# bcgsc/NanoSim

Hardware: NVIDIA H100
Metric: simulated_bases_per_sec (higher is better)
Workload: dtype u8

## Files before the change

### nanosim_b200/csrc/plan_kernel.cuh

```cuda
#pragma once
#include "device_common.cuh"

struct PlanArgs {
    DevModel m;
    DevRef ref;
    DevCfg cfg;
    uint32_t kind;
    uint64_t first_id;
    uint32_t n_reads;
    const uint32_t* n_seg;
    const uint32_t* piece_first;
    NsReadMeta* reads;
    NsPieceMeta* pieces;
    uint32_t* ops;
    const uint32_t* order;
    uint32_t* counter;
    uint32_t* n_flagged;
    uint32_t batch_reversed;
    const uint32_t* abort;
};

#define NS_MAX_SAME_LEN_RETRIES 64

enum Phase : int { PH_FETCH = 0, PH_LEN, PH_ATT, PH_PIECE, PH_EVENT, PH_UEVENT, PH_PIECE_END, PH_CHECK, PH_DONE };
// ... 94 lines not shown
}

__device__ __forceinline__ void draw_position_meta(const DevRef& ref, Rng& rng, int species, uint32_t length, uint32_t& chrom,
                                                   uint32_t& pos) {
    uint32_t sp = species >= 0 ? (uint32_t)species : (uint32_t)__umul64hi(rng.next64(), (uint64_t)ref.n_species);
    const uint32_t c0 = __ldg(&ref.species_chrom_off[sp]), c1 = __ldg(&ref.species_chrom_off[sp + 1]);
    uint32_t c = c0 + (uint32_t)__umul64hi(rng.next64(), (uint64_t)(c1 - c0));
    uint64_t clen = __ldg(&ref.chrom_off[c + 1]) - __ldg(&ref.chrom_off[c]);
    if ((uint64_t)length > clen) {
        uint32_t n_same = 0, n_all = 0;
        for (uint32_t q = 0; q < ref.n_chrom; ++q) {
            const uint64_t l = __ldg(&ref.chrom_off[q + 1]) - __ldg(&ref.chrom_off[q]);
            if ((uint64_t)length < l) {
                ++n_all;
                if (q >= c0 && q < c1) ++n_same;
            }
        }
        const bool same = n_same > 0;
        const uint32_t n_pick = same ? n_same : n_all - n_same;
        if (n_pick > 0) {
            uint32_t r = (uint32_t)__umul64hi(rng.next64(), (uint64_t)n_pick);
            for (uint32_t q = 0; q < ref.n_chrom; ++q) {
                const uint64_t l = __ldg(&ref.chrom_off[q + 1]) - __ldg(&ref.chrom_off[q]);
                const bool in_sp = q >= c0 && q < c1;
                if ((uint64_t)length < l && in_sp == same) {
                    if (r == 0) {
                        c = q;
                        break;
                    }
                    --r;
                }
            }
            clen = __ldg(&ref.chrom_off[c + 1]) - __ldg(&ref.chrom_off[c]);
        }
    }
    chrom = c;
    if (__ldg(&ref.chrom_circular[c])) {
        pos = (uint32_t)__umul64hi(rng.next64(), clen + 1);
    } else {
        pos = clen >= length ? (uint32_t)__umul64hi(rng.next64(), clen - length + 1) : 0u;
    }
}

__device__ __forceinline__ void draw_position_trx(const DevRef& ref, uint32_t n_records, Rng& rng, uint32_t length, uint32_t& chrom,
                                                  uint32_t& pos) {
    if (ref.trx_len_sorted && ref.n_trx_sorted == n_records) {
        uint32_t lo = 0, hi = n_records;
        while (lo < hi) {
            const uint32_t mid = (lo + hi) >> 1;
            if (__ldg(&ref.trx_len_sorted[mid]) > length) hi = mid; else lo = mid + 1;
        }
        if (lo < n_records) {
            const uint32_t j = lo + (uint32_t)__umul64hi(rng.next64(), (uint64_t)(n_records - lo));
            chrom = __ldg(&ref.trx_len_idx[j]);
            pos = (uint32_t)__umul64hi(rng.next64(), (uint64_t)(__ldg(&ref.trx_len_sorted[j]) - length + 1u));
            return;
        }
        chrom = 0;
        pos = 0;
        return;
    }
    for (int it = 0; it < 1000000; ++it) {
        const uint32_t c = (uint32_t)__umul64hi(rng.next64(), (uint64_t)n_records);
        const uint64_t clen = __ldg(&ref.chrom_off[c + 1]) - __ldg(&ref.chrom_off[c]);
        if ((uint64_t)length < clen) {
            chrom = c;
            pos = (uint32_t)__umul64hi(rng.next64(), clen - length + 1);
            return;
        }
    }
    chrom = 0;
    pos = 0;
}

__device__ __forceinline__ uint32_t lower_bound_f(const float* x, uint32_t n, float v) {
    uint32_t lo = 0, hi = n;
    while (lo < hi) {
        uint32_t mid = (lo + hi) >> 1;
        if (__ldg(&x[mid]) < v) lo = mid + 1; else hi = mid;
    }
    return lo;
}
__device__ __forceinline__ uint32_t nearest_aligned_length(const DevModel& m, uint32_t n_sample, uint32_t L, Rng& rng) {
    const uint32_t M = m.n_kde2d;
    const double u = u01_double(rng.next64());
    const double q = -expm1(log1p(-u) / (double)(n_sample > 0 ? n_sample : 1));
    const double need = q * (double)M;
    const float fl = (float)L;
    const float xmin = __ldg(&m.kde2d_x[0]), xmax = __ldg(&m.kde2d_x[M - 1]);
    uint32_t dlo = 0, dhi = (uint32_t)fmaxf(fabsf(fl - xmin), fabsf(xmax - fl)) + 1;
    while (dlo < dhi) {
        const uint32_t d = (dlo + dhi) >> 1;
        const uint32_t a = lower_bound_f(m.kde2d_x, M, fl - (float)d);
        const uint32_t b = lower_bound_f(m.kde2d_x, M, fl + (float)d + 0.5f);
        if ((double)(b - a) >= need && b > a) dhi = d; else dlo = d + 1;
    }
    const uint32_t d = dlo;
    const uint32_t a0 = lower_bound_f(m.kde2d_x, M, fl - (float)d), a1 = lower_bound_f(m.kde2d_x, M, fl - (float)d + 0.5f);
    uint32_t b0 = 0, b1 = 0;
    if (d > 0) {
        b0 = lower_bound_f(m.kde2d_x, M, fl + (float)d);
        b1 = lower_bound_f(m.kde2d_x, M, fl + (float)d + 0.5f);
    }
    const uint32_t cnt = (a1 - a0) + (b1 - b0);
    uint32_t r = (uint32_t)__umul64hi(rng.next64(), (uint64_t)(cnt > 0 ? cnt : 1));
    const uint32_t row = cnt == 0 ? (a0 < M ? a0 : M - 1) : (r < a1 - a0 ? a0 + r : b0 + (r - (a1 - a0)));
    const uint32_t r1 = rng.next(), r2 = rng.next();
    const float z = sqrtf(-2.0f * logf(u01_open_low(r1))) * cospif(2.0f * ((float)(r2 >> 8) * (1.0f / 16777216.0f)));
    const double y = (double)__ldg(&m.kde2d_y[row]) + (double)m.kde2d_bw * (double)z;
    return y > 0.0 ? (uint32_t)y : 0u;
}

__device__ __forceinline__ void draw_lengths(const DevModel& m, const DevCfg& cfg, uint32_t kind, uint64_t rid, uint32_t gen,
                                             uint32_t n_seg, NsPieceMeta* pieces) {
    Rng lr;
    lr.init(cfg.seed, rid, stream_word(ST_LEN, kind, gen));
    for (uint32_t s = 0; s < n_seg; ++s) {
        uint32_t len = 0;
        for (int it = 0; it < 100000; ++it) {
            double x;
            if (cfg.median_len > 0.0) {
                if (cfg.perfect) {
                    x = lognormal_draw(log(cfg.median_len), cfg.sd_len, lr);
                } else {
                    double t = lognormal_draw(log(cfg.median_len + cfg.sd_len * cfg.sd_len / 2.0), cfg.sd_len, lr);
                    double rem = -1.0;
                    for (int jt = 0; jt < 100000 && rem < 0.0; ++jt) rem = pow(10.0, kde_draw(m.ht, lr)) - 1.0;
                    x = t - rem;
                }
            } else {
                x = kde_draw(m.aligned, lr);
            }
            bool ok = cfg.perfect ? (x >= (double)cfg.min_len && x <= (double)cfg.max_len)
                                  : (x > 0.0 && x <= (double)cfg.max_len);
            if (cfg.metagenome) {
                if (ok) {
                    len = (uint32_t)rint(x);
                    break;
                }
                continue;
            }
            if (ok && (uint32_t)x > 0) {
                len = (uint32_t)x;
                break;
            }
        }
        pieces[2 * s].ref_req = len;
        if (s + 1 < n_seg) {
            double g = pow(10.0, kde_draw(m.gap, lr)) - 1.0;
            int64_t gi = (int64_t)g;
            pieces[2 * s + 1].ref_req = gi > 0 ? (uint32_t)gi : 0u;
        }
    }
}

__global__ void lengths_kernel(DevModel m, DevCfg cfg, uint32_t kind, uint64_t first_id, uint32_t n, const uint32_t* n_seg,
                               const uint32_t* piece_first, NsPieceMeta* pieces, float ev_per_base, float ev_cv, uint32_t exact_only,
                               uint64_t* caps, uint32_t* keys, uint32_t* vals) {
    uint32_t i = blockIdx.x * blockDim.x + threadIdx.x;
    if (i >= n) return;
    const uint32_t ns = n_seg ? n_seg[i] : 1u;
    const uint32_t pf = piece_first ? piece_first[i] : i;
    uint64_t total = 0;
    if (kind == NS_KIND_ALIGNED && cfg.transcriptome) {
        caps[pf] = 0;
    } else if (kind == NS_KIND_ALIGNED) {
        draw_lengths(m, cfg, kind, first_id + i, 0, ns, pieces + pf);
        for (uint32_t q = 0; q < 2 * ns - 1; ++q) {
            const uint32_t len = pieces[pf + q].ref_req;
            total += len;
            uint64_t cap;
            if (q & 1u) cap = 2ull * len + 64;
            else if (cfg.perfect) cap = 4;
            else {
                float e = (float)len * ev_per_base;
                cap = (uint64_t)(2.0f * (e + 6.0f * ev_cv * sqrtf(e) + 8.0f)) + 4;
            }
            caps[pf + q] = exact_only ? 0 : cap;
        }
    } else if (exact_only) {
        caps[pf] = 0;
    } else {
        Rng r0;
        r0.init(cfg.seed, first_id + i, stream_word(ST_ATT, NS_KIND_UNALIGNED, 0));
        const double x = cfg.median_len > 0.0 ? lognormal_draw(log(cfg.median_len), cfg.sd_len, r0) : kde_draw(m.unaligned, r0);
        const uint64_t len = x >= 1.0 ? (x < 268435455.0 ? (uint64_t)x : 268435455ull) : 0ull;
        caps[pf] = len + (len >> 1) + 64;
        total = len;
    }
    keys[i] = total > 0xffffffffull ? 0xffffffffu : (uint32_t)total;
    vals[i] = i;
}

#ifndef PLAN_MIN_BLOCKS
#define PLAN_MIN_BLOCKS 4
#endif
template <bool REPLAY>
__global__ void __launch_bounds__(128, PLAN_MIN_BLOCKS) plan_kernel(const __grid_constant__ PlanArgs a) {
    const DevModel& m = a.m;
    const DevCfg& cfg = a.cfg;
    const bool unal_kind = (a.kind == NS_KIND_UNALIGNED);
    if (a.abort && *a.abort) return;
    __shared__ uint8_t bin_lut[BIN_LUT_SIZE];
    __shared__ uint32_t s_tab_off[NS_MAX_TABLES], s_tab_n[NS_MAX_TABLES], s_trans[NS_N_ERR_STATES * 3];
    for (uint32_t i = threadIdx.x; i < BIN_LUT_SIZE; i += blockDim.x) bin_lut[i] = (uint8_t)match_bin_scan(m, i);
    for (uint32_t i = threadIdx.x; i < NS_MAX_TABLES; i += blockDim.x) {
        s_tab_off[i] = m.tab_off[i];
        s_tab_n[i] = m.tab_n[i];
    }
    for (uint32_t i = threadIdx.x; i < NS_N_ERR_STATES * 3; i += blockDim.x) s_trans[i] = m.trans[i / 3][i % 3];
    __syncthreads();

    int phase = PH_FETCH;
    uint32_t slot = 0;
    uint64_t rid = 0;
    uint32_t n_seg = 1, n_pieces = 1, piece_first = 0;
    uint32_t attempt = 0, gen = 0, gen_fails = 0;
    Rng rng;
    uint32_t remainder = 0, head = 0, tail = 0, reversed = 0;
    uint64_t total = 0, actual = 0;
    uint32_t p = 0;
    uint32_t pos = 0, middle_ref = 0, prev_match = 0, err_state = 0, last_err = 3;
    int64_t l_new = 0;
    uint32_t pending_ins = 0;
    uint4 ev_r = make_uint4(0, 0, 0, 0);
    uint32_t gap_sw = 0, gap_draw = 0;
    bool last_op_was_ins_same_pos = false;
    uint32_t last_ins_len = 0;
    OpSink<true> sink;
    sink.begin(nullptr, 0);
    bool overflow = false;

    for (;;) {
        switch (phase) {
        case PH_FETCH: {
            slot = atomicAdd(a.counter, 1u);
            if (slot >= a.n_reads) {
                phase = PH_DONE;
                break;
            }
            if (a.order) slot = a.order[slot];
            if (REPLAY && !(a.reads[slot].flags & 1u)) break;
            rid = a.first_id + slot;
            n_seg = a.n_seg ? a.n_seg[slot] : 1u;
            piece_first = a.piece_first ? a.piece_first[slot] : slot;
            n_pieces = unal_kind ? 1u : 2u * n_seg - 1u;
            overflow = false;
            if (REPLAY) {
                attempt = a.reads[slot].attempts;
            } else {
                attempt = 0;
                gen = 0;
                gen_fails = 0;
            }
            phase = PH_ATT;
            break;
        }
        case PH_LEN: {
            draw_lengths(m, cfg, a.kind, rid, gen, n_seg, a.pieces + piece_first);
            phase = PH_ATT;
            break;
        }
        case PH_ATT: {
            rng.init(cfg.seed, rid, stream_word(ST_ATT, a.kind, attempt));
            overflow = false;
            p = 0;
            total = 0;
            actual = 0;
            if (unal_kind) {
                double x = cfg.median_len > 0.0 ? lognormal_draw(log(cfg.median_len), cfg.sd_len, rng)
                                                : kde_draw(m.unaligned, rng);
                int64_t r = (int64_t)x;
                if (!REPLAY) a.pieces[piece_first].ref_req = r > 0 ? (uint32_t)r : 0u;
                head = tail = 0;
                remainder = 0;
                if (r <= 0 && !REPLAY) {
                    ++attempt;
                    break;
                }
            } else if (cfg.transcriptome) {
                uint32_t trx = 0, tlen = 0, alen = 0;
                for (int it = 0; it < 1000000; ++it) {
                    const uint32_t r = rng.next();
                    const uint64_t pp = (uint64_t)r * a.ref.n_expressed;
                    const uint32_t j = (uint32_t)(pp >> 32);
                    const uint2 e = __ldg(&a.ref.expr_alias[j]);
                    const uint32_t k = ((uint32_t)pp < e.x || e.x == 0xffffffffu) ? j : e.y;
                    trx = __ldg(&a.ref.expr_chrom[k]);
                    tlen = (uint32_t)(__ldg(&a.ref.chrom_off[trx + 1]) - __ldg(&a.ref.chrom_off[trx]));
                    alen = nearest_aligned_length(m, cfg.kde2d_n, tlen, rng);
                    if (alen < tlen) break;
                }
                NsPieceMeta& pm0 = a.pieces[piece_first];
                pm0.ref_req = alen;
                pm0.chrom = trx;
                reversed = u01_double(rng.next64()) > (double)m.strandness;
                head = tail = 0;
                remainder = 0;
                if (!cfg.perfect) {
                    Rng hr;
                    hr.init(cfg.seed, rid, stream_word(ST_LEN, a.kind, 0));
                    const double rem = pow(10.0, kde_draw(m.ht, hr)) - 1.0;
                    double ratio = kde_draw(m.ratio, hr);
                    ratio = ratio > 1.0 ? 1.0 : (ratio < 0.0 ? 0.0 : ratio);
                    remainder = rem > 0.0 ? (uint32_t)rem : 0u;
                    if (remainder > 0) {
                        head = (uint32_t)rint((double)remainder * ratio);
                        tail = remainder - head;
                    }
                }
            } else if (cfg.perfect) {
                head = tail = 0;
                remainder = 0;
                reversed = u01_double(rng.next64()) > (double)m.strandness;
                if (cfg.metagenome) reversed = a.batch_reversed;
            } else {
                double rem = -1.0;
                for (int it = 0; it < 100000 && rem < 0.0; ++it) rem = pow(10.0, kde_draw(m.ht, rng)) - 1.0;
                double ratio = -1.0;
                for (int it = 0; it < 100000 && (ratio < 0.0 || ratio > 1.0); ++it) ratio = kde_draw(m.ratio, rng);
                remainder = cfg.metagenome ? (uint32_t)rint(rem) : (uint32_t)rem;
                reversed = u01_double(rng.next64()) > (double)m.strandness;
                if (cfg.metagenome) reversed = a.batch_reversed;
                if (remainder == 0) {
                    head = tail = 0;
                } else {
                    head = (uint32_t)rint((double)remainder * ratio);
                    tail = remainder - head;
                }
                total = remainder;
            }
            phase = PH_PIECE;
            break;
        }
        case PH_PIECE: {
            NsPieceMeta& pm = a.pieces[piece_first + p];
            uint32_t m_ref = pm.ref_req;
            sink.begin(a.ops + pm.op_off, REPLAY ? 0xffffffffu : (uint32_t)(a.pieces[piece_first + p + 1].op_off - pm.op_off));
            pos = 0;
            middle_ref = m_ref;
            l_new = (int64_t)m_ref;
// ... 297 lines not shown
```

### nanosim_b200/csrc/uread_kernel.cuh

```cuda
#pragma once
#include "device_common.cuh"
#include "emit_kernel.cuh"
#include "plan_kernel.cuh"

struct UreadArgs {
    DevModel m;
    DevRef ref;
    DevCfg cfg;
    uint64_t first_id;
    uint32_t n_reads;
    NsReadMeta* reads;
    NsPieceMeta* pieces;
    uint32_t* ops;
    const uint32_t* order;
    uint32_t* counter;
    uint32_t* n_flagged;
    unsigned long long* pool_cursor;
    const uint64_t* pool;
    const uint32_t* abort;
    uint32_t cta_min_len;
};

#define UREAD_WARPS 8

__device__ __forceinline__ void scan_advance_and_insertions(bool nonins, uint32_t s, int lane, uint32_t& adv_incl, uint32_t& ins_incl) {
    if (__all_sync(0xffffffffu, s < 2048u)) {
        const uint32_t both = warp_incl_scan(nonins ? s : (s << 16), lane);
        adv_incl = both & 0xffffu;
        ins_incl = both >> 16;
    } else {
        adv_incl = warp_incl_scan(nonins ? s : 0u, lane);
        ins_incl = warp_incl_scan(nonins ? 0u : s, lane);
    }
}

struct UChain {
    uint32_t n_ops, middle_ref, n_draws;
    int64_t l_new;
};
__device__ __forceinline__ UChain unaligned_chain_warp(const DevModel& m, uint2 key, uint32_t id_lo, uint32_t id_hi, uint32_t sw,
                                                       uint32_t m_ref, uint32_t* ops, uint32_t cap, int lane) {
    const uint32_t lane_lt = (1u << lane) - 1u;
    uint32_t base = 0, pos_base = 0, carry_a = 0, middle_ref = m_ref, n_draws = 0, n_ops = 0;
    int64_t l_new = (int64_t)m_ref;
    bool done = false;
    auto draw = [&](uint32_t d, uint32_t& kd, uint32_t& sd) {
        const uint4 r = philox4x32_10(make_uint4(id_lo, id_hi, sw, d + 1u), key);
        kd = r.x < 1717986918u ? 0u : (r.x < 3006477107u ? 1u : (r.x < 3650722201u ? 2u : 3u));
        sd = 1;
        if (kd != 0) sd = alias_draw(m, kd == 1 ? 1u : (kd == 2 ? 2u : 3u), r.y);
    };
    uint32_t kind_next, s_next;
    draw(lane, kind_next, s_next);
    while (!done) {
        const uint32_t kind = kind_next, s = s_next;
        draw(base + 32u + lane, kind_next, s_next);
        const bool nonins = kind != 2;
        uint32_t Pl, I;
        scan_advance_and_insertions(nonins, s, lane, Pl, I);
        const uint32_t P = pos_base + Pl;
        const uint32_t stop_mask = __ballot_sync(0xffffffffu, nonins && P >= m_ref);
        const int jstop = stop_mask ? __ffs(stop_mask) - 1 : 32;
        const bool valid = lane <= jstop;
        const uint32_t nonins_mask = __ballot_sync(0xffffffffu, nonins);
        const uint32_t below = nonins_mask & lane_lt;
        const int pn = below ? 31 - __clz(below) : -1;
        const uint32_t I_pn = __shfl_sync(0xffffffffu, I, pn < 0 ? 0 : pn);
        const uint32_t a_ins = nonins ? (pn >= 0 ? I - I_pn : I + carry_a) : 0u;
        int32_t delta = 0;
        if (valid) delta = kind == 2 ? (int32_t)s : (kind == 3 ? -(int32_t)s : 0);
        delta = __reduce_add_sync(0xffffffffu, delta);
        l_new += delta;

        uint32_t o0 = 0, o1 = 0, o2 = 0, o3 = 0;
        const bool emits = valid && nonins;
        const uint32_t plain_mask = __ballot_sync(0xffffffffu, emits && kind == 0 && a_ins == 0);
        if (emits) {
            if (kind == 0) {
                if (a_ins == 0) {
                    if (!(lane > 0 && ((plain_mask >> (lane - 1)) & 1u))) {
                        const uint32_t run = __ffs(~(plain_mask >> lane)) - 1;
                        o0 = (NS_OP_COPY << 28) | (run == 0xffffffffu ? 32u - lane : run);
                    }
                } else {
                    o0 = (NS_OP_COPY << 28) | 1u;
                    o1 = (NS_OP_INS << 28) | a_ins;
                }
            } else {
                const uint32_t covered = a_ins < s - 1 ? a_ins : s - 1;
                const uint32_t rest = s - 1 - covered;
                const uint32_t T = kind == 1 ? NS_OP_MIS : NS_OP_DEL;
                const uint32_t n_ins = kind == 1 ? a_ins : a_ins - covered;
                if (n_ins == 0) {
                    o0 = (T << 28) | (1u + rest);
                } else {
                    o0 = (T << 28) | 1u;
                    o1 = (NS_OP_INS << 28) | n_ins;
                    if (rest) o2 = (T << 28) | rest;
                }
                if (covered) o3 = (NS_OP_COPY << 28) | covered;
            }
        }
        const uint32_t p1 = o0 ? 1u : 0u, p2 = p1 + (o1 ? 1u : 0u), p3 = p2 + (o2 ? 1u : 0u);
        const uint32_t cnt = p3 + (o3 ? 1u : 0u);
        const uint32_t incl = warp_incl_scan(cnt, lane);
        const uint32_t at = n_ops + incl - cnt;
        if (o0 && at < cap) ops[at] = o0;
        if (o1 && at + p1 < cap) ops[at + p1] = o1;
        if (o2 && at + p2 < cap) ops[at + p2] = o2;
        if (o3 && at + p3 < cap) ops[at + p3] = o3;
        n_ops += __shfl_sync(0xffffffffu, incl, 31);

        if (jstop < 32) {
            const uint32_t Pstop = __shfl_sync(0xffffffffu, P, jstop);
            if (Pstop > middle_ref) {
                l_new += Pstop - middle_ref;
                middle_ref = Pstop;
            }
            n_draws = base + (uint32_t)jstop + 1u;
            done = true;
        } else {
            pos_base = __shfl_sync(0xffffffffu, P, 31);
            const uint32_t I31 = __shfl_sync(0xffffffffu, I, 31);
            if (nonins_mask) {
                const int last = 31 - __clz(nonins_mask);
                carry_a = I31 - __shfl_sync(0xffffffffu, I, last);
            } else {
                carry_a += I31;
            }
            base += 32;
        }
    }
    UChain c;
    c.n_ops = n_ops;
    c.middle_ref = middle_ref;
    c.n_draws = n_draws;
    c.l_new = l_new;
    return c;
}


struct UCtaShared {
    uint32_t A[2][UREAD_WARPS], I[2][UREAD_WARPS], non[2][UREAD_WARPS], trail[2][UREAD_WARPS];
    uint32_t stop[2][UREAD_WARPS], cnt[2][UREAD_WARPS], pstop[2][UREAD_WARPS];
    int32_t delta[2][UREAD_WARPS];
    uint32_t bc32;
    unsigned long long bc64;
};
__device__ __forceinline__ UChain unaligned_chain_cta(const DevModel& m, uint2 key, uint32_t id_lo, uint32_t id_hi, uint32_t sw,
                                                      uint32_t m_ref, uint32_t* ops, uint32_t cap, UCtaShared& sh) {
    const int lane = threadIdx.x & 31, w = threadIdx.x >> 5;
    const uint32_t lane_lt = (1u << lane) - 1u;
    uint32_t base = 0, pos_base = 0, carry_round = 0, middle_ref = m_ref, n_draws = 0, n_ops = 0;
    int64_t l_new = (int64_t)m_ref;
    auto draw = [&](uint32_t d, uint32_t& kd, uint32_t& sd) {
        const uint4 r = philox4x32_10(make_uint4(id_lo, id_hi, sw, d + 1u), key);
        kd = r.x < 1717986918u ? 0u : (r.x < 3006477107u ? 1u : (r.x < 3650722201u ? 2u : 3u));
        sd = 1;
        if (kd != 0) sd = alias_draw(m, kd == 1 ? 1u : (kd == 2 ? 2u : 3u), r.y);
    };
    uint32_t kind_next, s_next;
    draw(32u * (uint32_t)w + lane, kind_next, s_next);
    for (uint32_t par = 0;; par ^= 1u) {
        const uint32_t kind = kind_next, s = s_next;
        draw(base + 32u * UREAD_WARPS + 32u * (uint32_t)w + lane, kind_next, s_next);
        const bool nonins = kind != 2;
        uint32_t Pl, I;
        scan_advance_and_insertions(nonins, s, lane, Pl, I);
        const uint32_t nonins_mask = __ballot_sync(0xffffffffu, nonins);
        const uint32_t P31 = __shfl_sync(0xffffffffu, Pl, 31), I31 = __shfl_sync(0xffffffffu, I, 31);
        const uint32_t I_last = __shfl_sync(0xffffffffu, I, nonins_mask ? 31 - __clz(nonins_mask) : 0);
        if (lane == 0) {
            sh.A[par][w] = P31;
            sh.I[par][w] = I31;
            sh.non[par][w] = nonins_mask != 0u;
            sh.trail[par][w] = nonins_mask ? I31 - I_last : I31;
        }
        __syncthreads();
        uint32_t pos_off = 0, carry_in = carry_round, A_tot = 0, carry_out = carry_round;
#pragma unroll
        for (int v = 0; v < UREAD_WARPS; ++v) {
            const uint32_t Av = sh.A[par][v];
            const uint32_t c = sh.non[par][v] ? sh.trail[par][v] : carry_out + sh.I[par][v];
            if (v < w) {
                pos_off += Av;
                carry_in = c;
            }
            carry_out = c;
            A_tot += Av;
        }
        const uint32_t P = pos_base + pos_off + Pl;
        const uint32_t stop_mask = __ballot_sync(0xffffffffu, nonins && P >= m_ref);
        const int jstop = stop_mask ? __ffs(stop_mask) - 1 : 32;
        const bool valid = lane <= jstop;
        const uint32_t below = nonins_mask & lane_lt;
        const int pn = below ? 31 - __clz(below) : -1;
        const uint32_t I_pn = __shfl_sync(0xffffffffu, I, pn < 0 ? 0 : pn);
        const uint32_t a_ins = nonins ? (pn >= 0 ? I - I_pn : I + carry_in) : 0u;
        int32_t delta = 0;
        if (valid) delta = kind == 2 ? (int32_t)s : (kind == 3 ? -(int32_t)s : 0);
        delta = __reduce_add_sync(0xffffffffu, delta);

        uint32_t o0 = 0, o1 = 0, o2 = 0, o3 = 0;
        const bool emits = valid && nonins;
        const uint32_t plain_mask = __ballot_sync(0xffffffffu, emits && kind == 0 && a_ins == 0);
        if (emits) {
            if (kind == 0) {
                if (a_ins == 0) {
                    if (!(lane > 0 && ((plain_mask >> (lane - 1)) & 1u))) {
                        const uint32_t run = __ffs(~(plain_mask >> lane)) - 1;
                        o0 = (NS_OP_COPY << 28) | (run == 0xffffffffu ? 32u - lane : run);
                    }
                } else {
                    o0 = (NS_OP_COPY << 28) | 1u;
                    o1 = (NS_OP_INS << 28) | a_ins;
                }
            } else {
                const uint32_t covered = a_ins < s - 1 ? a_ins : s - 1;
                const uint32_t rest = s - 1 - covered;
                const uint32_t T = kind == 1 ? NS_OP_MIS : NS_OP_DEL;
                const uint32_t n_ins = kind == 1 ? a_ins : a_ins - covered;
                if (n_ins == 0) {
                    o0 = (T << 28) | (1u + rest);
                } else {
                    o0 = (T << 28) | 1u;
                    o1 = (NS_OP_INS << 28) | n_ins;
                    if (rest) o2 = (T << 28) | rest;
                }
                if (covered) o3 = (NS_OP_COPY << 28) | covered;
            }
        }
        const uint32_t p1 = o0 ? 1u : 0u, p2 = p1 + (o1 ? 1u : 0u), p3 = p2 + (o2 ? 1u : 0u);
        const uint32_t cnt = p3 + (o3 ? 1u : 0u);
        const uint32_t incl = warp_incl_scan(cnt, lane);
        const uint32_t cnt_w = __shfl_sync(0xffffffffu, incl, 31);
        const uint32_t Pstop_w = __shfl_sync(0xffffffffu, P, jstop & 31);
        if (lane == 0) {
            sh.stop[par][w] = (uint32_t)jstop;
            sh.cnt[par][w] = cnt_w;
            sh.delta[par][w] = delta;
            sh.pstop[par][w] = Pstop_w;
        }
        __syncthreads();
        int ws = UREAD_WARPS;
#pragma unroll
        for (int v = UREAD_WARPS - 1; v >= 0; --v)
            if (sh.stop[par][v] < 32u) ws = v;
        uint32_t off = 0, tot = 0;
        int32_t dsum = 0;
#pragma unroll
        for (int v = 0; v < UREAD_WARPS; ++v) {
            if (v <= ws) {
                const uint32_t c = sh.cnt[par][v];
                if (v < w) off += c;
                tot += c;
                dsum += sh.delta[par][v];
            }
        }
        if (w <= ws) {
            const uint32_t at = n_ops + off + incl - cnt;
            if (o0 && at < cap) ops[at] = o0;
            if (o1 && at + p1 < cap) ops[at + p1] = o1;
            if (o2 && at + p2 < cap) ops[at + p2] = o2;
            if (o3 && at + p3 < cap) ops[at + p3] = o3;
        }
        n_ops += tot;
        l_new += dsum;
        if (ws < UREAD_WARPS) {
            const uint32_t Pstop = sh.pstop[par][ws];
            if (Pstop > middle_ref) {
                l_new += Pstop - middle_ref;
                middle_ref = Pstop;
            }
            n_draws = base + 32u * (uint32_t)ws + sh.stop[par][ws] + 1u;
            break;
        }
        pos_base += A_tot;
        carry_round = carry_out;
        base += 32u * UREAD_WARPS;
    }
    UChain c;
    c.n_ops = n_ops;
    c.middle_ref = middle_ref;
    c.n_draws = n_draws;
    c.l_new = l_new;
    return c;
}

#define UREAD_CTA_MIN_LEN 32768u

template <bool REPLAY, bool CTA>
__device__ __forceinline__ uint32_t uread_one(const UreadArgs& a, uint2 key, uint32_t slot, uint64_t pool_base, uint64_t pool_size,
                                              UCtaShared& sh) {
    const DevModel& m = a.m;
    const DevCfg& cfg = a.cfg;
    const int lane = threadIdx.x & 31;
    const bool leader = CTA ? threadIdx.x == 0 : lane == 0;
    const uint64_t rid = a.first_id + slot;
    const uint32_t id_lo = (uint32_t)rid, id_hi = (uint32_t)(rid >> 32);
    uint32_t attempt = REPLAY ? a.reads[slot].attempts : 0u;
    uint64_t op_off = a.pieces[slot].op_off;
    uint32_t* ops = a.ops + op_off;
    uint32_t cap = REPLAY ? 0xffffffffu : (uint32_t)(a.pieces[slot + 1].op_off - op_off);
    uint32_t first_len = 0;
    for (;;) {
        const uint32_t sw = stream_word(ST_ATT, NS_KIND_UNALIGNED, attempt);
        Rng r0;
        r0.init(cfg.seed, rid, sw);
        const double x = cfg.median_len > 0.0 ? lognormal_draw(log(cfg.median_len), cfg.sd_len, r0)
                                              : kde_draw(m.unaligned, r0);
        const int64_t mr = (int64_t)x;
        if (attempt == 0) first_len = mr > 0 ? (uint32_t)mr : 0u;
        if (mr <= 0) {
            ++attempt;
            continue;
        }
        const uint32_t m_ref = (uint32_t)mr;
        if (!REPLAY && attempt > 0) {
            const uint32_t need = m_ref + (m_ref >> 1) + 64u;
            unsigned long long off = 0;
            if (leader) off = atomicAdd(a.pool_cursor, (unsigned long long)need);
            if (CTA) {
                if (leader) sh.bc64 = off;
                __syncthreads();
                off = sh.bc64;
                __syncthreads();
            } else {
                off = __shfl_sync(0xffffffffu, off, 0);
            }
            if (off + need <= pool_size) {
                op_off = pool_base + off;
                cap = need;
            } else {
                cap = 0;
            }
            ops = a.ops + op_off;
        }
        const UChain ch = CTA ? unaligned_chain_cta(m, key, id_lo, id_hi, sw, m_ref, ops, cap, sh)
                              : unaligned_chain_warp(m, key, id_lo, id_hi, sw, m_ref, ops, cap, lane);
        const uint32_t middle_ref = ch.middle_ref, n_draws = ch.n_draws, n_ops = ch.n_ops;
        const int64_t l_new = ch.l_new;
        if (REPLAY) break;
        const bool ok = middle_ref >= cfg.min_len && middle_ref <= cfg.max_len && l_new >= (int64_t)cfg.min_len &&
                        l_new <= (int64_t)cfg.max_len;
        if (!ok) {
            ++attempt;
            continue;
        }
        const uint4 rs = philox4x32_10(make_uint4(id_lo, id_hi, sw, n_draws + 1u), key);
        const uint32_t reversed = u01_double(((uint64_t)rs.x << 32) | rs.y) > (double)m.strandness;
        Rng pr;
        pr.init(cfg.seed, rid, stream_word(ST_POS, NS_KIND_UNALIGNED, attempt));
        uint32_t chrom = 0, ppos = 0;
        if (cfg.metagenome) draw_position_meta(a.ref, pr, -1, middle_ref, chrom, ppos);
        else if (cfg.transcriptome) draw_position_trx(a.ref, cfg.trx_records ? cfg.trx_records : a.ref.n_chrom, pr, middle_ref, chrom, ppos);
        else draw_position(a.ref, cfg, pr, middle_ref, chrom, ppos);
        if (leader) {
            const bool overflow = n_ops > cap;
            NsPieceMeta p;
            p.op_off = op_off;
            p.n_ops = n_ops;
            p.kind = NS_PIECE_UNALIGNED;
            p.chrom = chrom;
            p.pos = ppos;
            p.ref_len = middle_ref;
            p.out_len = (uint32_t)l_new;
            p.out_rel = 0;
            p.l_new = (uint32_t)l_new;
            p.ref_req = m_ref;
            p.read_slot = slot;
            p.ev_off = op_off;
            p.ev_n_ops = n_ops;
            p.polya_len = 0;
            a.pieces[slot] = p;
            NsReadMeta q;
            q.seq_off = 0;
            q.seq_len = (uint32_t)l_new;
            q.head = 0;
            q.tail = 0;
            q.piece_first = slot;
            q.n_pieces = 1;
            q.reversed = (uint8_t)reversed;
            q.flags = overflow ? 1 : 0;
            q.attempts = attempt;
            a.reads[slot] = q;
            if (overflow) atomicAdd(a.n_flagged, 1u);
        }
        break;
    }
    return first_len;
}

#ifndef UREAD_MIN_BLOCKS
#define UREAD_MIN_BLOCKS 3
#endif
template <bool REPLAY>
__global__ void __launch_bounds__(UREAD_WARPS * 32, UREAD_MIN_BLOCKS) uread_kernel(const __grid_constant__ UreadArgs a) {
    const int lane = threadIdx.x & 31;
    const uint2 key = make_uint2((uint32_t)a.cfg.seed, (uint32_t)(a.cfg.seed >> 32));
    if (a.abort && *a.abort) return;
    const uint64_t pool_base = a.pool[0], pool_size = a.pool[1];
    __shared__ UCtaShared sh;

    if (!REPLAY && a.order && a.cta_min_len) {
        for (;;) {
            if (threadIdx.x == 0) sh.bc32 = atomicAdd(a.counter, 1u);
            __syncthreads();
            const uint32_t idx = sh.bc32;
            __syncthreads();
            if (idx >= a.n_reads) return;
            const uint32_t first_len = uread_one<REPLAY, true>(a, key, a.order[idx], pool_base, pool_size, sh);
            if (first_len <= a.cta_min_len) break;
        }
    }
    for (;;) {
        uint32_t idx = 0;
        if (lane == 0) idx = atomicAdd(a.counter, 1u);
        idx = __shfl_sync(0xffffffffu, idx, 0);
        if (idx >= a.n_reads) break;
        const uint32_t slot = a.order ? a.order[idx] : idx;
        if (REPLAY && !(a.reads[slot].flags & 1u)) continue;
        uread_one<REPLAY, false>(a, key, slot, pool_base, pool_size, sh);
    }
}

struct GapArgs {
    DevModel m;
    DevCfg cfg;
    uint32_t kind;
    uint64_t first_id;
    uint32_t n_reads;
    const uint32_t* n_seg;
    const uint32_t* piece_first;
    NsPieceMeta* pieces;
    uint32_t* ops;
    uint32_t* counter;
    const uint32_t* abort;
};
__device__ __forceinline__ uint32_t gap_stream_word(uint32_t kind, uint32_t attempt, uint32_t piece_in_read) {
    return stream_word(ST_GAP, kind, (attempt << 5) | (piece_in_read & 31u));
}
__global__ void __launch_bounds__(UREAD_WARPS * 32) gap_kernel(const __grid_constant__ GapArgs a) {
    const int lane = threadIdx.x & 31;
    const uint2 key = make_uint2((uint32_t)a.cfg.seed, (uint32_t)(a.cfg.seed >> 32));
    if (a.abort && *a.abort) return;
    for (;;) {
        uint32_t slot = 0;
        if (lane == 0) slot = atomicAdd(a.counter, 1u);
        slot = __shfl_sync(0xffffffffu, slot, 0);
        if (slot >= a.n_reads) break;
        const uint32_t ns = a.n_seg[slot];
        if (ns < 2) continue;
        const uint32_t pf = a.piece_first[slot];
        const uint64_t rid = a.first_id + slot;
        for (uint32_t q = 1; q < 2 * ns - 1; q += 2) {
            NsPieceMeta& pm = a.pieces[pf + q];
            const uint32_t m_ref = pm.ref_req;
            if (m_ref == 0) continue;
            const uint64_t op_off = pm.op_off;
            const uint32_t cap = (uint32_t)(a.pieces[pf + q + 1].op_off - op_off);
            const UChain ch = unaligned_chain_warp(a.m, key, (uint32_t)rid, (uint32_t)(rid >> 32), gap_stream_word(a.kind, 0, q), m_ref,
                                                   a.ops + op_off, cap, lane);
            if (lane == 0) {
                pm.n_ops = ch.n_ops;
                pm.ref_len = ch.middle_ref;
                pm.out_len = (uint32_t)(ch.l_new < 0 ? 0 : ch.l_new);
                pm.l_new = pm.out_len;
                pm.polya_len = 1;
            }
        }
    }
}
```

Before: 122.2 billion.

## Process four error draws per lane in unaligned chain and unify warp/CTA paths

Each lane now handles four consecutive error-model draws instead of one. The lane scans its draws locally and the warp/CTA scans run over per-lane aggregates, so shuffle, ballot and sync overhead is spread across more work per round. The warp and CTA chain variants are merged into one template, alias-table lookups are inlined with hoisted table offsets, and min blocks drops to 2 to allow more registers. The CTA-vs-warp switch and the sort key now use the total length over retried attempts, which costs extra length draws per read.

```diff
diff --git a/nanosim_b200/csrc/plan_kernel.cuh b/nanosim_b200/csrc/plan_kernel.cuh
--- a/nanosim_b200/csrc/plan_kernel.cuh
+++ b/nanosim_b200/csrc/plan_kernel.cuh
@@ -270,6 +270,22 @@
             pieces[2 * s + 1].ref_req = gi > 0 ? (uint32_t)gi : 0u;
         }
     }
+}
+
+__device__ __forceinline__ uint64_t unaligned_len(const DevModel& m, const DevCfg& cfg, uint64_t rid, uint32_t attempt) {
+    Rng r0;
+    r0.init(cfg.seed, rid, stream_word(ST_ATT, NS_KIND_UNALIGNED, attempt));
+    const double x = cfg.median_len > 0.0 ? lognormal_draw(log(cfg.median_len), cfg.sd_len, r0) : kde_draw(m.unaligned, r0);
+    return x >= 1.0 ? (x < 268435455.0 ? (uint64_t)x : 268435455ull) : 0ull;
+}
+__device__ __forceinline__ uint32_t unaligned_work(const DevModel& m, const DevCfg& cfg, uint64_t rid) {
+    uint64_t work = 0;
+    for (uint32_t attempt = 0; attempt < 16; ++attempt) {
+        const uint64_t len = unaligned_len(m, cfg, rid, attempt);
+        work += len;
+        if (len >= cfg.min_len) break;
+    }
+    return work > 0xffffffffull ? 0xffffffffu : (uint32_t)work;
 }
 
 __global__ void lengths_kernel(DevModel m, DevCfg cfg, uint32_t kind, uint64_t first_id, uint32_t n, const uint32_t* n_seg,
@@ -299,12 +315,9 @@
     } else if (exact_only) {
         caps[pf] = 0;
     } else {
-        Rng r0;
-        r0.init(cfg.seed, first_id + i, stream_word(ST_ATT, NS_KIND_UNALIGNED, 0));
-        const double x = cfg.median_len > 0.0 ? lognormal_draw(log(cfg.median_len), cfg.sd_len, r0) : kde_draw(m.unaligned, r0);
-        const uint64_t len = x >= 1.0 ? (x < 268435455.0 ? (uint64_t)x : 268435455ull) : 0ull;
+        const uint64_t len = unaligned_len(m, cfg, first_id + i, 0);
         caps[pf] = len + (len >> 1) + 64;
-        total = len;
+        total = unaligned_work(m, cfg, first_id + i);
     }
     keys[i] = total > 0xffffffffull ? 0xffffffffu : (uint32_t)total;
     vals[i] = i;
diff --git a/nanosim_b200/csrc/uread_kernel.cuh b/nanosim_b200/csrc/uread_kernel.cuh
--- a/nanosim_b200/csrc/uread_kernel.cuh
+++ b/nanosim_b200/csrc/uread_kernel.cuh
@@ -22,15 +22,65 @@
 };
 
 #define UREAD_WARPS 8
-
-__device__ __forceinline__ void scan_advance_and_insertions(bool nonins, uint32_t s, int lane, uint32_t& adv_incl, uint32_t& ins_incl) {
-    if (__all_sync(0xffffffffu, s < 2048u)) {
-        const uint32_t both = warp_incl_scan(nonins ? s : (s << 16), lane);
+#define UREAD_DRAWS 4
+#define UREAD_WARP_DRAWS (32u * UREAD_DRAWS)
+static_assert(UREAD_DRAWS == 4, "a 32-draw group (a COPY run's limit) is the 8 lanes 8g .. 8g+7");
+
+struct UTabs {
+    const uint2* alias;
+    uint32_t off1, off2, off3, n1, n2, n3;
+};
+__device__ __forceinline__ UTabs utabs(const DevModel& m) {
+    UTabs t;
+    t.alias = m.alias;
+    t.off1 = m.tab_off[1], t.off2 = m.tab_off[2], t.off3 = m.tab_off[3];
+    t.n1 = m.tab_n[1], t.n2 = m.tab_n[2], t.n3 = m.tab_n[3];
+    return t;
+}
+
+__device__ __forceinline__ uint32_t udraw(const UTabs& tb, uint2 key, uint32_t id_lo, uint32_t id_hi, uint32_t sw, uint32_t d) {
+    const uint4 r = philox4x32_10(make_uint4(id_lo, id_hi, sw, d + 1u), key);
+    const uint32_t kd = r.x < 1717986918u ? 0u : (r.x < 3006477107u ? 1u : (r.x < 3650722201u ? 2u : 3u));
+    const uint32_t n = kd <= 1 ? tb.n1 : (kd == 2 ? tb.n2 : tb.n3), off = kd <= 1 ? tb.off1 : (kd == 2 ? tb.off2 : tb.off3);
+    const uint64_t p = (uint64_t)r.y * n;
+    const uint32_t j = (uint32_t)(p >> 32);
+    const uint2 e = __ldg(&tb.alias[off + j]);
+    const uint32_t sd = kd == 0 ? 1u : (((uint32_t)p < e.x || e.x == 0xffffffffu) ? j : e.y);
+    return (kd << 30) | sd;
+}
+__device__ __forceinline__ uint32_t ukind(uint32_t d) { return d >> 30; }
+__device__ __forceinline__ uint32_t ulen(uint32_t d) { return d & 0x3fffffffu; }
+
+__device__ __forceinline__ void udraw_ops(uint32_t kind, uint32_t s, uint32_t a_ins, uint32_t& o0, uint32_t& o1, uint32_t& o2,
+                                          uint32_t& o3) {
+    o0 = o1 = o2 = o3 = 0;
+    if (kind == 0) {
+        o0 = (NS_OP_COPY << 28) | 1u;
+        o1 = (NS_OP_INS << 28) | a_ins;
+    } else {
+        const uint32_t covered = a_ins < s - 1 ? a_ins : s - 1;
+        const uint32_t rest = s - 1 - covered;
+        const uint32_t T = kind == 1 ? NS_OP_MIS : NS_OP_DEL;
+        const uint32_t n_ins = kind == 1 ? a_ins : a_ins - covered;
+        if (n_ins == 0) {
+            o0 = (T << 28) | (1u + rest);
+        } else {
+            o0 = (T << 28) | 1u;
+            o1 = (NS_OP_INS << 28) | n_ins;
+            if (rest) o2 = (T << 28) | rest;
+        }
+        if (covered) o3 = (NS_OP_COPY << 28) | covered;
+    }
+}
+
+__device__ __forceinline__ void scan_advance_and_insertions(uint32_t adv, uint32_t ins, int lane, uint32_t& adv_incl, uint32_t& ins_incl) {
+    if (__all_sync(0xffffffffu, adv < 2048u && ins < 2048u)) {
+        const uint32_t both = warp_incl_scan(adv | (ins << 16), lane);
         adv_incl = both & 0xffffu;
         ins_incl = both >> 16;
     } else {
-        adv_incl = warp_incl_scan(nonins ? s : 0u, lane);
-        ins_incl = warp_incl_scan(nonins ? 0u : s, lane);
+        adv_incl = warp_incl_scan(adv, lane);
+        ins_incl = warp_incl_scan(ins, lane);
     }
 }
 
@@ -38,107 +88,6 @@
     uint32_t n_ops, middle_ref, n_draws;
     int64_t l_new;
 };
-__device__ __forceinline__ UChain unaligned_chain_warp(const DevModel& m, uint2 key, uint32_t id_lo, uint32_t id_hi, uint32_t sw,
-                                                       uint32_t m_ref, uint32_t* ops, uint32_t cap, int lane) {
-    const uint32_t lane_lt = (1u << lane) - 1u;
-    uint32_t base = 0, pos_base = 0, carry_a = 0, middle_ref = m_ref, n_draws = 0, n_ops = 0;
-    int64_t l_new = (int64_t)m_ref;
-    bool done = false;
-    auto draw = [&](uint32_t d, uint32_t& kd, uint32_t& sd) {
-        const uint4 r = philox4x32_10(make_uint4(id_lo, id_hi, sw, d + 1u), key);
-        kd = r.x < 1717986918u ? 0u : (r.x < 3006477107u ? 1u : (r.x < 3650722201u ? 2u : 3u));
-        sd = 1;
-        if (kd != 0) sd = alias_draw(m, kd == 1 ? 1u : (kd == 2 ? 2u : 3u), r.y);
-    };
-    uint32_t kind_next, s_next;
-    draw(lane, kind_next, s_next);
-    while (!done) {
-        const uint32_t kind = kind_next, s = s_next;
-        draw(base + 32u + lane, kind_next, s_next);
-        const bool nonins = kind != 2;
-        uint32_t Pl, I;
-        scan_advance_and_insertions(nonins, s, lane, Pl, I);
-        const uint32_t P = pos_base + Pl;
-        const uint32_t stop_mask = __ballot_sync(0xffffffffu, nonins && P >= m_ref);
-        const int jstop = stop_mask ? __ffs(stop_mask) - 1 : 32;
-        const bool valid = lane <= jstop;
-        const uint32_t nonins_mask = __ballot_sync(0xffffffffu, nonins);
-        const uint32_t below = nonins_mask & lane_lt;
-        const int pn = below ? 31 - __clz(below) : -1;
-        const uint32_t I_pn = __shfl_sync(0xffffffffu, I, pn < 0 ? 0 : pn);
-        const uint32_t a_ins = nonins ? (pn >= 0 ? I - I_pn : I + carry_a) : 0u;
-        int32_t delta = 0;
-        if (valid) delta = kind == 2 ? (int32_t)s : (kind == 3 ? -(int32_t)s : 0);
-        delta = __reduce_add_sync(0xffffffffu, delta);
-        l_new += delta;
-
-        uint32_t o0 = 0, o1 = 0, o2 = 0, o3 = 0;
-        const bool emits = valid && nonins;
-        const uint32_t plain_mask = __ballot_sync(0xffffffffu, emits && kind == 0 && a_ins == 0);
-        if (emits) {
-            if (kind == 0) {
-                if (a_ins == 0) {
-                    if (!(lane > 0 && ((plain_mask >> (lane - 1)) & 1u))) {
-                        const uint32_t run = __ffs(~(plain_mask >> lane)) - 1;
-                        o0 = (NS_OP_COPY << 28) | (run == 0xffffffffu ? 32u - lane : run);
-                    }
-                } else {
-                    o0 = (NS_OP_COPY << 28) | 1u;
-                    o1 = (NS_OP_INS << 28) | a_ins;
-                }
-            } else {
-                const uint32_t covered = a_ins < s - 1 ? a_ins : s - 1;
-                const uint32_t rest = s - 1 - covered;
-                const uint32_t T = kind == 1 ? NS_OP_MIS : NS_OP_DEL;
-                const uint32_t n_ins = kind == 1 ? a_ins : a_ins - covered;
-                if (n_ins == 0) {
-                    o0 = (T << 28) | (1u + rest);
-                } else {
-                    o0 = (T << 28) | 1u;
-                    o1 = (NS_OP_INS << 28) | n_ins;
-                    if (rest) o2 = (T << 28) | rest;
-                }
-                if (covered) o3 = (NS_OP_COPY << 28) | covered;
-            }
-        }
-        const uint32_t p1 = o0 ? 1u : 0u, p2 = p1 + (o1 ? 1u : 0u), p3 = p2 + (o2 ? 1u : 0u);
-        const uint32_t cnt = p3 + (o3 ? 1u : 0u);
-        const uint32_t incl = warp_incl_scan(cnt, lane);
-        const uint32_t at = n_ops + incl - cnt;
-        if (o0 && at < cap) ops[at] = o0;
-        if (o1 && at + p1 < cap) ops[at + p1] = o1;
-        if (o2 && at + p2 < cap) ops[at + p2] = o2;
-        if (o3 && at + p3 < cap) ops[at + p3] = o3;
-        n_ops += __shfl_sync(0xffffffffu, incl, 31);
-
-        if (jstop < 32) {
-            const uint32_t Pstop = __shfl_sync(0xffffffffu, P, jstop);
-            if (Pstop > middle_ref) {
-                l_new += Pstop - middle_ref;
-                middle_ref = Pstop;
-            }
-            n_draws = base + (uint32_t)jstop + 1u;
-            done = true;
-        } else {
-            pos_base = __shfl_sync(0xffffffffu, P, 31);
-            const uint32_t I31 = __shfl_sync(0xffffffffu, I, 31);
-            if (nonins_mask) {
-                const int last = 31 - __clz(nonins_mask);
-                carry_a = I31 - __shfl_sync(0xffffffffu, I, last);
-            } else {
-                carry_a += I31;
-            }
-            base += 32;
-        }
-    }
-    UChain c;
-    c.n_ops = n_ops;
-    c.middle_ref = middle_ref;
-    c.n_draws = n_draws;
-    c.l_new = l_new;
-    return c;
-}
-
 
 struct UCtaShared {
     uint32_t A[2][UREAD_WARPS], I[2][UREAD_WARPS], non[2][UREAD_WARPS], trail[2][UREAD_WARPS];
@@ -147,137 +96,205 @@
     uint32_t bc32;
     unsigned long long bc64;
 };
-__device__ __forceinline__ UChain unaligned_chain_cta(const DevModel& m, uint2 key, uint32_t id_lo, uint32_t id_hi, uint32_t sw,
-                                                      uint32_t m_ref, uint32_t* ops, uint32_t cap, UCtaShared& sh) {
-    const int lane = threadIdx.x & 31, w = threadIdx.x >> 5;
+
+template <bool CTA>
+__device__ __forceinline__ UChain unaligned_chain(const UTabs& tb, uint2 key, uint32_t id_lo, uint32_t id_hi, uint32_t sw, uint32_t m_ref,
+                                                 uint32_t* ops, uint32_t cap, UCtaShared* sh) {
+    constexpr uint32_t ROUND = CTA ? UREAD_WARP_DRAWS * UREAD_WARPS : UREAD_WARP_DRAWS;
+    const int lane = threadIdx.x & 31, w = CTA ? (int)(threadIdx.x >> 5) : 0;
     const uint32_t lane_lt = (1u << lane) - 1u;
-    uint32_t base = 0, pos_base = 0, carry_round = 0, middle_ref = m_ref, n_draws = 0, n_ops = 0;
+    const uint32_t first = UREAD_WARP_DRAWS * (uint32_t)w + UREAD_DRAWS * (uint32_t)lane;
+    uint32_t base = 0, pos_base = 0, carry = 0, middle_ref = m_ref, n_draws = 0, n_ops = 0;
     int64_t l_new = (int64_t)m_ref;
-    auto draw = [&](uint32_t d, uint32_t& kd, uint32_t& sd) {
-        const uint4 r = philox4x32_10(make_uint4(id_lo, id_hi, sw, d + 1u), key);
-        kd = r.x < 1717986918u ? 0u : (r.x < 3006477107u ? 1u : (r.x < 3650722201u ? 2u : 3u));
-        sd = 1;
-        if (kd != 0) sd = alias_draw(m, kd == 1 ? 1u : (kd == 2 ? 2u : 3u), r.y);
-    };
-    uint32_t kind_next, s_next;
-    draw(32u * (uint32_t)w + lane, kind_next, s_next);
+    uint32_t nxt[UREAD_DRAWS];
+#pragma unroll
+    for (int k = 0; k < UREAD_DRAWS; ++k) nxt[k] = udraw(tb, key, id_lo, id_hi, sw, first + k);
     for (uint32_t par = 0;; par ^= 1u) {
-        const uint32_t kind = kind_next, s = s_next;
-        draw(base + 32u * UREAD_WARPS + 32u * (uint32_t)w + lane, kind_next, s_next);
-        const bool nonins = kind != 2;
-        uint32_t Pl, I;
-        scan_advance_and_insertions(nonins, s, lane, Pl, I);
-        const uint32_t nonins_mask = __ballot_sync(0xffffffffu, nonins);
-        const uint32_t P31 = __shfl_sync(0xffffffffu, Pl, 31), I31 = __shfl_sync(0xffffffffu, I, 31);
-        const uint32_t I_last = __shfl_sync(0xffffffffu, I, nonins_mask ? 31 - __clz(nonins_mask) : 0);
-        if (lane == 0) {
-            sh.A[par][w] = P31;
-            sh.I[par][w] = I31;
-            sh.non[par][w] = nonins_mask != 0u;
-            sh.trail[par][w] = nonins_mask ? I31 - I_last : I31;
-        }
-        __syncthreads();
-        uint32_t pos_off = 0, carry_in = carry_round, A_tot = 0, carry_out = carry_round;
-#pragma unroll
-        for (int v = 0; v < UREAD_WARPS; ++v) {
-            const uint32_t Av = sh.A[par][v];
-            const uint32_t c = sh.non[par][v] ? sh.trail[par][v] : carry_out + sh.I[par][v];
-            if (v < w) {
-                pos_off += Av;
-                carry_in = c;
-            }
-            carry_out = c;
-            A_tot += Av;
-        }
-        const uint32_t P = pos_base + pos_off + Pl;
-        const uint32_t stop_mask = __ballot_sync(0xffffffffu, nonins && P >= m_ref);
-        const int jstop = stop_mask ? __ffs(stop_mask) - 1 : 32;
-        const bool valid = lane <= jstop;
-        const uint32_t below = nonins_mask & lane_lt;
+        uint32_t dr[UREAD_DRAWS];
+#pragma unroll
+        for (int k = 0; k < UREAD_DRAWS; ++k) {
+            dr[k] = nxt[k];
+            nxt[k] = udraw(tb, key, id_lo, id_hi, sw, base + ROUND + first + k);
+        }
+        uint32_t adv = 0, ins = 0, trail = 0;
+        bool has_non = false;
+#pragma unroll
+        for (int k = 0; k < UREAD_DRAWS; ++k) {
+            const uint32_t s = ulen(dr[k]);
+            if (ukind(dr[k]) == 2) {
+                ins += s;
+                trail += s;
+            } else {
+                adv += s;
+                trail = 0;
+                has_non = true;
+            }
+        }
+        uint32_t adv_incl, ins_incl;
+        scan_advance_and_insertions(adv, ins, lane, adv_incl, ins_incl);
+        const uint32_t non_mask = __ballot_sync(0xffffffffu, has_non);
+        const uint32_t X = ins_incl - trail;
+        const uint32_t A31 = __shfl_sync(0xffffffffu, adv_incl, 31), I31 = __shfl_sync(0xffffffffu, ins_incl, 31);
+        const uint32_t X_last = __shfl_sync(0xffffffffu, X, non_mask ? 31 - __clz(non_mask) : 0);
+        uint32_t pos_off = 0, carry_in = carry, A_tot = A31, carry_out = non_mask ? I31 - X_last : carry + I31;
+        if constexpr (CTA) {
+            if (lane == 0) {
+                sh->A[par][w] = A31;
+                sh->I[par][w] = I31;
+                sh->non[par][w] = non_mask != 0u;
+                sh->trail[par][w] = non_mask ? I31 - X_last : I31;
+            }
+            __syncthreads();
+            A_tot = 0;
+            carry_out = carry;
+#pragma unroll
+            for (int v = 0; v < UREAD_WARPS; ++v) {
+                const uint32_t Av = sh->A[par][v];
+                const uint32_t c = sh->non[par][v] ? sh->trail[par][v] : carry_out + sh->I[par][v];
+                if (v < w) {
+                    pos_off += Av;
+                    carry_in = c;
+                }
+                carry_out = c;
+                A_tot += Av;
+            }
+        }
+        uint32_t p = pos_base + pos_off + adv_incl - adv, pstop = 0;
+        int kst = UREAD_DRAWS;
+#pragma unroll
+        for (int k = 0; k < UREAD_DRAWS; ++k) {
+            if (ukind(dr[k]) != 2) {
+                p += ulen(dr[k]);
+                if (kst == UREAD_DRAWS && p >= m_ref) {
+                    kst = k;
+                    pstop = p;
+                }
+            }
+        }
+        const uint32_t stop_mask = __ballot_sync(0xffffffffu, kst < UREAD_DRAWS);
+        const int jl = stop_mask ? __ffs(stop_mask) - 1 : 32;
+        const int n_valid = lane < jl ? UREAD_DRAWS : (lane == jl ? kst + 1 : 0);
+        const uint32_t below = non_mask & lane_lt;
         const int pn = below ? 31 - __clz(below) : -1;
-        const uint32_t I_pn = __shfl_sync(0xffffffffu, I, pn < 0 ? 0 : pn);
-        const uint32_t a_ins = nonins ? (pn >= 0 ? I - I_pn : I + carry_in) : 0u;
+        const uint32_t X_pn = __shfl_sync(0xffffffffu, X, pn < 0 ? 0 : pn);
+        const uint32_t a_first = ins_incl - ins + (pn >= 0 ? 0u - X_pn : carry_in);
+
+        uint32_t plain = 0, cnt = 0, a_ins = a_first;
         int32_t delta = 0;
-        if (valid) delta = kind == 2 ? (int32_t)s : (kind == 3 ? -(int32_t)s : 0);
-        delta = __reduce_add_sync(0xffffffffu, delta);
-
-        uint32_t o0 = 0, o1 = 0, o2 = 0, o3 = 0;
-        const bool emits = valid && nonins;
-        const uint32_t plain_mask = __ballot_sync(0xffffffffu, emits && kind == 0 && a_ins == 0);
-        if (emits) {
-            if (kind == 0) {
-                if (a_ins == 0) {
-                    if (!(lane > 0 && ((plain_mask >> (lane - 1)) & 1u))) {
-                        const uint32_t run = __ffs(~(plain_mask >> lane)) - 1;
-                        o0 = (NS_OP_COPY << 28) | (run == 0xffffffffu ? 32u - lane : run);
-                    }
+#pragma unroll
+        for (int k = 0; k < UREAD_DRAWS; ++k) {
+            const uint32_t kind = ukind(dr[k]), s = ulen(dr[k]);
+            if (kind == 2) {
+                a_ins += s;
+                if (k < n_valid) delta += (int32_t)s;
+                continue;
+            }
+            if (k < n_valid) {
+                if (kind == 3) delta -= (int32_t)s;
+                if (kind == 0 && a_ins == 0) {
+                    plain |= 1u << k;
                 } else {
-                    o0 = (NS_OP_COPY << 28) | 1u;
-                    o1 = (NS_OP_INS << 28) | a_ins;
-                }
-            } else {
-                const uint32_t covered = a_ins < s - 1 ? a_ins : s - 1;
-                const uint32_t rest = s - 1 - covered;
-                const uint32_t T = kind == 1 ? NS_OP_MIS : NS_OP_DEL;
-                const uint32_t n_ins = kind == 1 ? a_ins : a_ins - covered;
-                if (n_ins == 0) {
-                    o0 = (T << 28) | (1u + rest);
-                } else {
-                    o0 = (T << 28) | 1u;
-                    o1 = (NS_OP_INS << 28) | n_ins;
-                    if (rest) o2 = (T << 28) | rest;
-                }
-                if (covered) o3 = (NS_OP_COPY << 28) | covered;
-            }
-        }
-        const uint32_t p1 = o0 ? 1u : 0u, p2 = p1 + (o1 ? 1u : 0u), p3 = p2 + (o2 ? 1u : 0u);
-        const uint32_t cnt = p3 + (o3 ? 1u : 0u);
+                    uint32_t o0, o1, o2, o3;
+                    udraw_ops(kind, s, a_ins, o0, o1, o2, o3);
+                    cnt += (o0 ? 1u : 0u) + (o1 ? 1u : 0u) + (o2 ? 1u : 0u) + (o3 ? 1u : 0u);
+                }
+            }
+            a_ins = 0;
+        }
+        const uint32_t last_mask = __ballot_sync(0xffffffffu, (plain >> (UREAD_DRAWS - 1)) & 1u);
+        const uint32_t full_mask = __ballot_sync(0xffffffffu, plain == (1u << UREAD_DRAWS) - 1u);
+        const bool cont = (lane & 7) != 0 && ((last_mask >> ((lane - 1) & 31)) & 1u);
+        const uint32_t starts = plain & ~((plain << 1) | (cont ? 1u : 0u));
+        cnt += __popc(starts);
+        const int gend = lane | 7;
+        const uint32_t after = ~full_mask & ((2u << gend) - 1u) & ~((2u << lane) - 1u);
+        const int t = after ? __ffs(after) - 1 : gend + 1;
+        const uint32_t lead_t = __shfl_sync(0xffffffffu, (uint32_t)__ffs(~plain) - 1u, t & 31);
+        const uint32_t run_on = UREAD_DRAWS * (uint32_t)(t - lane - 1) + (after ? lead_t : 0u);
+
         const uint32_t incl = warp_incl_scan(cnt, lane);
         const uint32_t cnt_w = __shfl_sync(0xffffffffu, incl, 31);
-        const uint32_t Pstop_w = __shfl_sync(0xffffffffu, P, jstop & 31);
-        if (lane == 0) {
-            sh.stop[par][w] = (uint32_t)jstop;
-            sh.cnt[par][w] = cnt_w;
-            sh.delta[par][w] = delta;
-            sh.pstop[par][w] = Pstop_w;
-        }
-        __syncthreads();
-        int ws = UREAD_WARPS;
-#pragma unroll
-        for (int v = UREAD_WARPS - 1; v >= 0; --v)
-            if (sh.stop[par][v] < 32u) ws = v;
-        uint32_t off = 0, tot = 0;
-        int32_t dsum = 0;
-#pragma unroll
-        for (int v = 0; v < UREAD_WARPS; ++v) {
-            if (v <= ws) {
-                const uint32_t c = sh.cnt[par][v];
-                if (v < w) off += c;
-                tot += c;
-                dsum += sh.delta[par][v];
-            }
-        }
-        if (w <= ws) {
-            const uint32_t at = n_ops + off + incl - cnt;
-            if (o0 && at < cap) ops[at] = o0;
-            if (o1 && at + p1 < cap) ops[at + p1] = o1;
-            if (o2 && at + p2 < cap) ops[at + p2] = o2;
-            if (o3 && at + p3 < cap) ops[at + p3] = o3;
+        const int32_t delta_w = __reduce_add_sync(0xffffffffu, delta);
+        const uint32_t kst_w = __shfl_sync(0xffffffffu, (uint32_t)kst, jl & 31);
+        const uint32_t Pstop_w = __shfl_sync(0xffffffffu, pstop, jl & 31);
+        const uint32_t stop_w = jl < 32 ? UREAD_DRAWS * (uint32_t)jl + kst_w : UREAD_WARP_DRAWS;
+        uint32_t off = 0, tot = cnt_w, stop_r = stop_w, Pstop = Pstop_w;
+        int32_t dsum = delta_w;
+        bool writes = true;
+        if constexpr (CTA) {
+            if (lane == 0) {
+                sh->stop[par][w] = stop_w;
+                sh->cnt[par][w] = cnt_w;
+                sh->delta[par][w] = delta_w;
+                sh->pstop[par][w] = Pstop_w;
+            }
+            __syncthreads();
+            int ws = UREAD_WARPS;
+#pragma unroll
+            for (int v = UREAD_WARPS - 1; v >= 0; --v)
+                if (sh->stop[par][v] < UREAD_WARP_DRAWS) ws = v;
+            tot = 0;
+            dsum = 0;
+#pragma unroll
+            for (int v = 0; v < UREAD_WARPS; ++v) {
+                if (v <= ws) {
+                    const uint32_t c = sh->cnt[par][v];
+                    if (v < w) off += c;
+                    tot += c;
+                    dsum += sh->delta[par][v];
+                }
+            }
+            writes = w <= ws;
+            stop_r = ws < UREAD_WARPS ? UREAD_WARP_DRAWS * (uint32_t)ws + sh->stop[par][ws] : ROUND;
+            if (ws < UREAD_WARPS) Pstop = sh->pstop[par][ws];
+        }
+
+        if (writes) {
+            uint32_t at = n_ops + off + incl - cnt;
+            a_ins = a_first;
+#pragma unroll
+            for (int k = 0; k < UREAD_DRAWS; ++k) {
+                const uint32_t kind = ukind(dr[k]), s = ulen(dr[k]);
+                if (kind == 2) {
+                    a_ins += s;
+                    continue;
+                }
+                if (k < n_valid) {
+                    if ((plain >> k) & 1u) {
+                        if ((starts >> k) & 1u) {
+                            uint32_t run = __ffs(~(plain >> k)) - 1;
+                            if (k + run == UREAD_DRAWS) run += run_on;
+                            if (at < cap) ops[at] = (NS_OP_COPY << 28) | run;
+                            ++at;
+                        }
+                    } else {
+                        uint32_t o[4];
+                        udraw_ops(kind, s, a_ins, o[0], o[1], o[2], o[3]);
+#pragma unroll
+                        for (int i = 0; i < 4; ++i) {
+                            if (o[i]) {
+                                if (at < cap) ops[at] = o[i];
+                                ++at;
+                            }
+                        }
+                    }
+                }
+                a_ins = 0;
+            }
         }
         n_ops += tot;
         l_new += dsum;
-        if (ws < UREAD_WARPS) {
-            const uint32_t Pstop = sh.pstop[par][ws];
+        if (stop_r < ROUND) {
             if (Pstop > middle_ref) {
                 l_new += Pstop - middle_ref;
                 middle_ref = Pstop;
             }
-            n_draws = base + 32u * (uint32_t)ws + sh.stop[par][ws] + 1u;
+            n_draws = base + stop_r + 1u;
             break;
         }
         pos_base += A_tot;
-        carry_round = carry_out;
-        base += 32u * UREAD_WARPS;
+        carry = carry_out;
+        base += ROUND;
     }
     UChain c;
     c.n_ops = n_ops;
@@ -290,8 +307,8 @@
 #define UREAD_CTA_MIN_LEN 32768u
 
 template <bool REPLAY, bool CTA>
-__device__ __forceinline__ uint32_t uread_one(const UreadArgs& a, uint2 key, uint32_t slot, uint64_t pool_base, uint64_t pool_size,
-                                              UCtaShared& sh) {
+__device__ __forceinline__ void uread_one(const UreadArgs& a, const UTabs& tb, uint2 key, uint32_t slot, uint64_t pool_base,
+                                              uint64_t pool_size, UCtaShared& sh) {
     const DevModel& m = a.m;
     const DevCfg& cfg = a.cfg;
     const int lane = threadIdx.x & 31;
@@ -302,7 +319,6 @@
     uint64_t op_off = a.pieces[slot].op_off;
     uint32_t* ops = a.ops + op_off;
     uint32_t cap = REPLAY ? 0xffffffffu : (uint32_t)(a.pieces[slot + 1].op_off - op_off);
-    uint32_t first_len = 0;
     for (;;) {
         const uint32_t sw = stream_word(ST_ATT, NS_KIND_UNALIGNED, attempt);
         Rng r0;
@@ -310,7 +326,6 @@
         const double x = cfg.median_len > 0.0 ? lognormal_draw(log(cfg.median_len), cfg.sd_len, r0)
                                               : kde_draw(m.unaligned, r0);
         const int64_t mr = (int64_t)x;
-        if (attempt == 0) first_len = mr > 0 ? (uint32_t)mr : 0u;
         if (mr <= 0) {
             ++attempt;
             continue;
@@ -336,8 +351,7 @@
             }
             ops = a.ops + op_off;
         }
-        const UChain ch = CTA ? unaligned_chain_cta(m, key, id_lo, id_hi, sw, m_ref, ops, cap, sh)
-                              : unaligned_chain_warp(m, key, id_lo, id_hi, sw, m_ref, ops, cap, lane);
+        const UChain ch = unaligned_chain<CTA>(tb, key, id_lo, id_hi, sw, m_ref, ops, cap, &sh);
         const uint32_t middle_ref = ch.middle_ref, n_draws = ch.n_draws, n_ops = ch.n_ops;
         const int64_t l_new = ch.l_new;
         if (REPLAY) break;
@@ -388,11 +402,10 @@
         }
         break;
     }
-    return first_len;
 }
 
 #ifndef UREAD_MIN_BLOCKS
-#define UREAD_MIN_BLOCKS 3
+#define UREAD_MIN_BLOCKS 2
 #endif
 template <bool REPLAY>
 __global__ void __launch_bounds__(UREAD_WARPS * 32, UREAD_MIN_BLOCKS) uread_kernel(const __grid_constant__ UreadArgs a) {
@@ -400,6 +413,7 @@
     const uint2 key = make_uint2((uint32_t)a.cfg.seed, (uint32_t)(a.cfg.seed >> 32));
     if (a.abort && *a.abort) return;
     const uint64_t pool_base = a.pool[0], pool_size = a.pool[1];
+    const UTabs tb = utabs(a.m);
     __shared__ UCtaShared sh;
 
     if (!REPLAY && a.order && a.cta_min_len) {
@@ -409,8 +423,9 @@
             const uint32_t idx = sh.bc32;
             __syncthreads();
             if (idx >= a.n_reads) return;
-            const uint32_t first_len = uread_one<REPLAY, true>(a, key, a.order[idx], pool_base, pool_size, sh);
-            if (first_len <= a.cta_min_len) break;
+            const uint32_t slot = a.order[idx];
+            uread_one<REPLAY, true>(a, tb, key, slot, pool_base, pool_size, sh);
+            if (unaligned_work(a.m, a.cfg, a.first_id + slot) <= a.cta_min_len) break;
         }
     }
     for (;;) {
@@ -420,7 +435,7 @@
         if (idx >= a.n_reads) break;
         const uint32_t slot = a.order ? a.order[idx] : idx;
         if (REPLAY && !(a.reads[slot].flags & 1u)) continue;
-        uread_one<REPLAY, false>(a, key, slot, pool_base, pool_size, sh);
+        uread_one<REPLAY, false>(a, tb, key, slot, pool_base, pool_size, sh);
     }
 }
 
@@ -444,6 +459,7 @@
     const int lane = threadIdx.x & 31;
     const uint2 key = make_uint2((uint32_t)a.cfg.seed, (uint32_t)(a.cfg.seed >> 32));
     if (a.abort && *a.abort) return;
+    const UTabs tb = utabs(a.m);
     for (;;) {
         uint32_t slot = 0;
         if (lane == 0) slot = atomicAdd(a.counter, 1u);
@@ -459,8 +475,8 @@
             if (m_ref == 0) continue;
             const uint64_t op_off = pm.op_off;
             const uint32_t cap = (uint32_t)(a.pieces[pf + q + 1].op_off - op_off);
-            const UChain ch = unaligned_chain_warp(a.m, key, (uint32_t)rid, (uint32_t)(rid >> 32), gap_stream_word(a.kind, 0, q), m_ref,
-                                                   a.ops + op_off, cap, lane);
+            const UChain ch = unaligned_chain<false>(tb, key, (uint32_t)rid, (uint32_t)(rid >> 32), gap_stream_word(a.kind, 0, q), m_ref,
+                                                     a.ops + op_off, cap, nullptr);
             if (lane == 0) {
                 pm.n_ops = ch.n_ops;
                 pm.ref_len = ch.middle_ref;
```

After: 123.5 billion, median of 6. About the same (+1.0%).
